# FoundationVision/OmniTokenizer

Measured on NVIDIA H100. Metric: video_frames_per_sec_encode_decode, higher is better.
Workload: dtype f32

## Files before the change

omnitokenizer_b200/_cabi.py:

```python
from __future__ import annotations

import ctypes
import os
from ctypes import c_char_p, c_float, c_int, c_int64, c_void_p, POINTER

import torch

_LIB_NAME = "libomnitok_b200.so"
_lib = None

EPI_NONE, EPI_GEGLU, EPI_QKV, EPI_QKV_PLANES = 0, 1, 2, 3
MATH_FP32, MATH_3XTF32, MATH_F16X1, MATH_F16X3 = 0, 1, 2, 3
ABI_VERSION = 2


class LinearHArgs(ctypes.Structure):
    _fields_ = [("a_hi", c_void_p), ("a_lo", c_void_p), ("a_rs", c_void_p), ("a2_rs", c_void_p), ("w_scale", c_float),
                ("a2_hi", c_void_p), ("a2_lo", c_void_p), ("n_split", c_int),
                ("lda", c_int), ("a_seg", c_int), ("a_seg_stride", c_int), ("a_seg_off", c_int),
                ("w_hi", c_void_p), ("w_lo", c_void_p),
                ("c", c_void_p), ("ldc", c_int), ("c_seg", c_int), ("c_seg_stride", c_int), ("c_seg_off", c_int),
                ("u_hi", c_void_p), ("u_lo", c_void_p), ("ldu", c_int),
                ("M", c_int), ("N", c_int), ("K", c_int),
                ("bias", c_void_p), ("residual", c_void_p), ("ldr", c_int),
                ("epilogue", c_int),
                ("q_scale", c_void_p), ("k_scale", c_void_p), ("rope_cos", c_void_p), ("rope_sin", c_void_p),
                ("qk_cols", c_int), ("tokens", c_int),
                ("q_plane_scale", c_float), ("k_plane_scale", c_float), ("vinv", c_void_p),
                ("a_rs_uniform", c_float), ("u_scale", c_float)]


SIGNATURES = {
    "omt_abi_version": (c_int, []),
    "omt_last_error": (c_char_p, []),
    "omt_device_info": (c_int, [POINTER(c_int)] * 3),
    "omt_set_option": (c_int, [c_char_p, c_int]),
    "omt_linear": (c_int, [c_void_p, c_int, c_int, c_int, c_int, c_void_p, c_void_p, c_void_p, c_int, c_int, c_int,
                           c_int, c_int, c_int, c_int, c_void_p, c_void_p, c_int, c_int, c_int, c_void_p]),
    "omt_linear2": (c_int, [c_void_p, c_void_p, c_int, c_int, c_void_p, c_void_p, c_void_p, c_int, c_int, c_int, c_int,
                            c_int, c_void_p, c_void_p, c_void_p, c_void_p, c_int, c_int, c_void_p]),
    "omt_linear_h": (c_int, [POINTER(LinearHArgs), c_void_p]),
    "omt_linear_h1": (c_int, [POINTER(LinearHArgs), c_void_p]),
    "omt_layernorm": (c_int, [c_void_p, c_int, c_void_p, c_int, c_void_p, c_void_p, c_int, c_int, c_float, c_int, c_int,
                              c_int, c_void_p]),
    "omt_layernorm_h": (c_int, [c_void_p, c_int, c_void_p, c_int, c_void_p, c_void_p, c_void_p, c_void_p, c_void_p, c_void_p,
                                c_int, c_void_p, c_void_p, c_int, c_int, c_float, c_int, c_int, c_int, c_void_p]),
    "omt_patchify_ln": (c_int, [c_void_p, c_void_p, c_void_p, c_void_p, c_void_p, c_void_p, c_void_p] + [c_int] * 8 + [c_float, c_void_p]),
    "omt_patchify_ln_u8": (c_int, [c_void_p] * 9 + [c_int] * 8 + [c_float, c_void_p]),
    "omt_u8_norm_select": (c_int, [c_void_p, c_int, c_int64, c_void_p, c_void_p]),
    "omt_resample_u8": (c_int, [c_void_p, c_int64, c_void_p, c_void_p, c_void_p, c_void_p, c_int64, c_int, c_int, c_int,
                                c_void_p, c_void_p]),
    "omt_resample_clips": (c_int, [c_void_p, c_int64, c_void_p, c_void_p, c_void_p, c_void_p, c_int64, c_void_p, c_int,
                                   c_int, c_int, c_int, c_void_p, c_void_p]),
    "omt_fvd_preprocess": (c_int, [c_void_p, c_int64, c_void_p, c_void_p, c_void_p, c_void_p, c_int64, c_void_p,
                                   c_void_p, c_int, c_int, c_int, c_int, c_void_p, c_void_p]),
    "omt_fvd_suite_preprocess": (c_int, [c_void_p, c_int64, c_int, c_int, c_void_p, c_void_p, c_void_p, c_void_p,
                                         c_int64, c_int, c_int, c_int, c_int, c_void_p, c_void_p]),
    "omt_conv3d": (c_int, [c_void_p, c_int, c_int, c_int, c_int, c_int, c_void_p, c_void_p, c_int, c_void_p]
                   + [c_int] * 13 + [c_void_p, c_int, c_int, c_void_p]),
    "omt_maxpool3d": (c_int, [c_void_p] + [c_int] * 17 + [c_void_p, c_void_p]),
    "omt_i3d_head": (c_int, [c_void_p, c_int, c_int, c_int, c_int, c_void_p, c_void_p, c_int, c_void_p, c_void_p]),
    "omt_fid_preprocess": (c_int, [c_void_p, c_int64, c_void_p, c_void_p, c_void_p, c_void_p, c_int64, c_void_p,
                                   c_void_p, c_int, c_int, c_int, c_void_p, c_void_p]),
    "omt_pool2d": (c_int, [c_void_p] + [c_int] * 13 + [c_void_p, c_int, c_int, c_void_p]),
    "omt_psnr_ssim": (c_int, [c_void_p] * 6 + [c_int] * 4 + [c_void_p] * 4),
    "omt_lpips_input": (c_int, [c_void_p] * 4 + [c_int] * 4 + [c_void_p, c_void_p]),
    "omt_lpips_head": (c_int, [c_void_p] + [c_int] * 5 + [c_void_p, c_int, c_void_p, c_void_p, c_void_p]),
    "omt_unpatchify": (c_int, [c_void_p, c_void_p] + [c_int] * 8 + [c_void_p]),
    "omt_unpatchify_u8": (c_int, [c_void_p, c_void_p] + [c_int] * 8 + [c_float] * 5 + [c_void_p]),
    "omt_peg": (c_int, [c_void_p, c_void_p, c_void_p, c_void_p, c_void_p, c_int, c_int, c_int, c_void_p]),
    "omt_peg_volume": (c_int, [c_void_p, c_void_p, c_void_p, c_void_p] + [c_int] * 7 + [c_void_p]),
    "omt_peg_volume_varlen": (c_int, [c_void_p] * 6 + [c_int] * 7 + [c_void_p]),
    "omt_qk_prep": (c_int, [c_void_p, c_int, c_void_p, c_int, c_void_p, c_void_p, c_void_p, c_void_p, c_int, c_int,
                            c_int, c_void_p]),
    "omt_attn_spatial": (c_int, [c_void_p, c_int, c_void_p, c_int, c_void_p, c_int, c_void_p, c_void_p, c_void_p, c_int,
                                 c_int, c_int, c_int, c_float, c_void_p]),
    "omt_attn_spatial_h": (c_int, [c_void_p, c_void_p, c_int, c_void_p, c_void_p, c_int, c_void_p, c_void_p, c_int, c_void_p,
                                   c_float, c_void_p, c_void_p, c_void_p, c_int, c_int, c_int, c_int, c_float, c_void_p]),
    "omt_attn_spatial_h1": (c_int, [c_void_p, c_int, c_void_p, c_int, c_void_p, c_int, c_void_p, c_float, c_void_p, c_void_p,
                                    c_int, c_int, c_int, c_int, c_float, c_void_p]),
    "omt_attn_window": (c_int, [c_void_p, c_int, c_void_p, c_int, c_void_p, c_int, c_void_p, c_void_p, c_void_p, c_int,
                                c_void_p, c_int, c_int, c_int, c_int, c_int, c_float, c_void_p]),
    "omt_attn_temporal": (c_int, [c_void_p, c_int, c_void_p, c_int, c_void_p, c_int, c_void_p, c_void_p, c_void_p, c_int,
                                  c_int, c_int, c_int, c_int, c_float, c_int, c_void_p]),
    "omt_attn_temporal_varlen": (c_int, [c_void_p, c_int, c_void_p, c_int, c_void_p, c_int, c_void_p, c_void_p, c_void_p,
                                         c_int, c_void_p, c_void_p, c_int, c_int, c_int, c_int, c_float, c_int, c_void_p]),
    "omt_pre_vq": (c_int, [c_void_p, c_int, c_void_p, c_void_p, c_void_p, c_int, c_int, c_int, c_int, c_void_p]),
    "omt_vq_search": (c_int, [c_void_p, c_void_p, c_void_p, c_int, c_int, c_void_p, c_void_p, c_void_p]),
    "omt_vq_fused": (c_int, [c_void_p, c_int, c_void_p, c_void_p, c_int, c_int, c_void_p, c_void_p, c_void_p, c_int, c_int,
                             c_void_p, c_void_p, c_void_p]),
    "omt_post_vq": (c_int, [c_void_p] * 8 + [c_int, c_int, c_int, c_void_p]),
}


def lib_path() -> str:
    return os.environ.get("OMT_LIB") or os.path.join(os.path.dirname(os.path.abspath(__file__)), _LIB_NAME)


def load():
    global _lib
    if _lib is not None:
        return _lib
    path = lib_path()
    if not os.path.exists(path):
        raise RuntimeError(
            f"{path} not found: the CUDA extension is not built. Run `python -c 'import __graft_entry__ as g; "
            f"g.build()'` (or `make -C omnitokenizer_b200/csrc`). There is no CPU fallback.")
    lib = ctypes.CDLL(path)
    for name, (res, args) in SIGNATURES.items():
        fn = getattr(lib, name)
        fn.restype = res
        fn.argtypes = args
    if lib.omt_abi_version() != ABI_VERSION:
        raise RuntimeError("libomnitok_b200.so ABI version mismatch")
    _lib = lib
    return lib


def _ptr(t):
    if t is None:
        return None
    if isinstance(t, int):
        return t
    return t.data_ptr()


def _stream():
    return torch.cuda.current_stream().cuda_stream


KERNELS_PER_CALL = {"omt_u8_norm_select": 2}
launch_count = 0


def call(name: str, *args):
    global launch_count
    lib = load()
    launch_count += KERNELS_PER_CALL.get(name, 1)
    conv = [_ptr(a) if (a is None or isinstance(a, torch.Tensor)) else a for a in args]
    rc = getattr(lib, name)(*conv, _stream())
    if rc != 0:
        raise RuntimeError(f"{name} failed ({rc}): {lib.omt_last_error().decode()}")


def linear_h(name="omt_linear_h", **kw):
    global launch_count
    lib = load()
    a = LinearHArgs()
    for k, v in kw.items():
        setattr(a, k, _ptr(v) if (v is None or isinstance(v, torch.Tensor)) else v)
    launch_count += 1
    rc = getattr(lib, name)(ctypes.byref(a), _stream())
    if rc != 0:
        raise RuntimeError(f"{name} failed ({rc}): {lib.omt_last_error().decode()}")


DEFAULT_OPTIONS = {"attn_kernel": 3, "peg_kernel": 4, "f16_bn": 0, "attn_f16_ctas": 2}


def set_option(name: str, value: int):
    lib = load()
    rc = lib.omt_set_option(name.encode(), int(value))
    if rc != 0:
        raise RuntimeError(f"omt_set_option({name}) failed: {lib.omt_last_error().decode()}")


def device_info():
    lib = load()
    a, b, c = c_int(), c_int(), c_int()
    rc = lib.omt_device_info(ctypes.byref(a), ctypes.byref(b), ctypes.byref(c))
    if rc != 0:
        raise RuntimeError(lib.omt_last_error().decode())
    return a.value, b.value, c.value
```

omnitokenizer_b200/csrc/rowwise.cu:

```cuda
#include "omt_common.cuh"
#include <string.h>

namespace omt {

static thread_local char g_err[512] = "";

void set_error(const char* fmt, ...) {
  va_list ap;
  va_start(ap, fmt);
  vsnprintf(g_err, sizeof(g_err), fmt, ap);
  va_end(ap);
}

int g_peg_kernel = 4;
int g_pdl = 0;
static int g_dev_ok[64];
static int g_sms[64];

int check_device() {
  int dev = 0;
  OMT_CUDA(cudaGetDevice(&dev));
  if (dev < 0 || dev >= 64) { set_error("device ordinal %d out of range", dev); return OMT_E_ARG; }
  if (g_dev_ok[dev] == 0) {
    cudaDeviceProp p;
    OMT_CUDA(cudaGetDeviceProperties(&p, dev));
    g_sms[dev] = p.multiProcessorCount;
    g_dev_ok[dev] = (p.major == 9 && p.minor == 0) ? 1 : -1;
  }
  if (g_dev_ok[dev] < 0) {
    set_error("omnitok_b200 kernels are built for sm_90a (H100) only (no fallback path)");
    return OMT_E_ARCH;
  }
  return OMT_OK;
}

int sm_count() {
  int dev = 0;
  cudaGetDevice(&dev);
  return (dev >= 0 && dev < 64 && g_sms[dev] > 0) ? g_sms[dev] : 148;
}

struct LnPlanes {
  uint16_t* y_hi; uint16_t* y_lo;
  uint16_t* x_hi; uint16_t* x_lo;
  int lds;
  float* y_rs; float* x_rs;
};

template <int NV, bool PAIR>
__global__ void __launch_bounds__(256) layernorm_kernel(const float* __restrict__ x, int ldx,
                                                        float* __restrict__ y, int ldy,
                                                        const float* __restrict__ w,
                                                        const float* __restrict__ b, int M, int C,
                                                        float eps, int seg, int seg_stride, int seg_off,
                                                        const LnPlanes pl) {
  pdl_sync();
  const int lane = threadIdx.x & 31;
  const int lrow = blockIdx.x * (blockDim.x >> 5) + (threadIdx.x >> 5);
  if (lrow >= M) return;
  const long long row = map_row(lrow, seg, seg_stride, seg_off);
  const float* xr = x + (size_t)row * ldx;
  float4 v[NV];
  float s = 0.f;
#pragma unroll
  for (int i = 0; i < NV; ++i) {
    const int c = PAIR ? ((i >> 1) * 32 + lane) * 8 + (i & 1) * 4 : (i * 32 + lane) * 4;
    if (c < C) {
      v[i] = *reinterpret_cast<const float4*>(xr + c);
      s += (v[i].x + v[i].y) + (v[i].z + v[i].w);
      if (pl.x_hi != nullptr && pl.x_rs == nullptr) store_split4(pl.x_hi, pl.x_lo, (size_t)lrow * pl.lds + c, v[i]);
    } else {
      v[i] = make_float4(0.f, 0.f, 0.f, 0.f);
    }
  }
  if (pl.x_hi != nullptr && pl.x_rs != nullptr) {
    float mx = 0.f;
#pragma unroll
    for (int i = 0; i < NV; ++i) mx = fmaxf(mx, max4abs(v[i]));
    float sc, inv;
    row_scale(warp_max(mx), sc, inv);
    if constexpr (PAIR) {
#pragma unroll
      for (int i = 0; i < NV; i += 2) {
        const int c = ((i >> 1) * 32 + lane) * 8;
        if (c < C) store_split8u(pl.x_hi, pl.x_lo, (size_t)lrow * pl.lds + c, v[i], v[i + 1], sc);
      }
    } else {
#pragma unroll
      for (int i = 0; i < NV; ++i) {
        const int c = (i * 32 + lane) * 4;
        if (c < C) store_split4u(pl.x_hi, pl.x_lo, (size_t)lrow * pl.lds + c, v[i], sc);
      }
    }
    if (lane == 0) pl.x_rs[lrow] = inv;
  }
  const float mean = warp_sum(s) / (float)C;
  float q = 0.f;
#pragma unroll
  for (int i = 0; i < NV; ++i) {
    const int c = PAIR ? ((i >> 1) * 32 + lane) * 8 + (i & 1) * 4 : (i * 32 + lane) * 4;
    if (c < C) {
      v[i].x -= mean; v[i].y -= mean; v[i].z -= mean; v[i].w -= mean;
      q += (v[i].x * v[i].x + v[i].y * v[i].y) + (v[i].z * v[i].z + v[i].w * v[i].w);
    }
  }
  const float rstd = 1.0f / sqrtf(warp_sum(q) / (float)C + eps);
  float* yr = y + (size_t)row * ldy;
  float omx = 0.f;
#pragma unroll
  for (int i = 0; i < NV; ++i) {
    const int c = PAIR ? ((i >> 1) * 32 + lane) * 8 + (i & 1) * 4 : (i * 32 + lane) * 4;
    if (c < C) {
      const float4 g = *reinterpret_cast<const float4*>(w + c);
      float4 o;
      o.x = v[i].x * rstd * g.x; o.y = v[i].y * rstd * g.y;
      o.z = v[i].z * rstd * g.z; o.w = v[i].w * rstd * g.w;
      if (b != nullptr) {
        const float4 bb = *reinterpret_cast<const float4*>(b + c);
        o.x += bb.x; o.y += bb.y; o.z += bb.z; o.w += bb.w;
      }
      if (y != nullptr) *reinterpret_cast<float4*>(yr + c) = o;
      if (pl.y_hi != nullptr && pl.y_rs == nullptr) store_split4(pl.y_hi, pl.y_lo, (size_t)lrow * pl.lds + c, o);
      v[i] = o;
      omx = fmaxf(omx, max4abs(o));
    }
  }
  if (pl.y_hi != nullptr && pl.y_rs != nullptr) {
    float sc, inv;
    row_scale(warp_max(omx), sc, inv);
    if constexpr (PAIR) {
#pragma unroll
      for (int i = 0; i < NV; i += 2) {
        const int c = ((i >> 1) * 32 + lane) * 8;
        if (c < C) store_split8u(pl.y_hi, pl.y_lo, (size_t)lrow * pl.lds + c, v[i], v[i + 1], sc);
      }
    } else {
#pragma unroll
      for (int i = 0; i < NV; ++i) {
        const int c = (i * 32 + lane) * 4;
        if (c < C) store_split4u(pl.y_hi, pl.y_lo, (size_t)lrow * pl.lds + c, v[i], sc);
      }
    }
    if (lane == 0) pl.y_rs[lrow] = inv;
  }
}

struct PatchRow {
  int bi, t0, hi, wi;
};

__device__ __forceinline__ PatchRow patch_row(int row, int T, int H, int W, int p, int pt, int first) {
  const int hh = H / p, ww = W / p;
  int r = row;
  PatchRow pr;
  pr.wi = r % ww; r /= ww;
  pr.hi = r % hh; r /= hh;
  int ti = 0;
  if (!first) { const int tn = (T - 1) / pt; ti = r % tn; r /= tn; }
  pr.bi = r;
  pr.t0 = first ? 0 : 1 + ti * pt;
  return pr;
}

template <int NV>
__device__ __forceinline__ void patch_ln_emit(float4 (&v)[NV], int row, int K, int lane, float* __restrict__ A,
                                              uint16_t* __restrict__ A_hi, uint16_t* __restrict__ A_lo,
                                              float* __restrict__ A_rs, const float* __restrict__ lw,
// ... 343 lines not shown
#pragma unroll
  for (int r9 = 0; r9 < 9; ++r9) {
    const float* rp = tp + ((st + r9 / 3) * (HB + 2) + sh + r9 % 3) * RS;
    win[r9][1] = *reinterpret_cast<const float2*>(rp);
    win[r9][2] = *reinterpret_cast<const float2*>(rp + PEG_CC);
  }
  const int fbase = ((t0 + st) * h + (h0 + sh)) * w;
  int tau = fbase % T, nn = fbase / T;
  for (int w2 = 0; w2 < w; ++w2) {
    float2 acc = bb;
#pragma unroll
    for (int r9 = 0; r9 < 9; ++r9) {
      const float* rp = tp + ((st + r9 / 3) * (HB + 2) + sh + r9 % 3) * RS + (w2 + 2) * PEG_CC;
      win[r9][0] = win[r9][1]; win[r9][1] = win[r9][2];
      win[r9][2] = *reinterpret_cast<const float2*>(rp);
#pragma unroll
      for (int kw = 0; kw < 3; ++kw) {
        acc.x = fmaf(win[r9][kw].x, wt[r9 * 3 + kw].x, acc.x);
        acc.y = fmaf(win[r9][kw].y, wt[r9 * 3 + kw].y, acc.y);
      }
    }
    const float2 ctr = causal ? win[7][1] : win[4][1];
    acc.x += ctr.x; acc.y += ctr.y;
    const int row = temporal ? tau * N + nn : fbase + w2;
    *reinterpret_cast<float2*>(y + (bbase + row) * C + c0 + 2 * cp) = acc;
    if (++tau == T) { tau = 0; ++nn; }
  }
}

__device__ __forceinline__ float2 lds_f2(uint32_t addr) {
  float2 v;
  asm volatile("ld.shared.v2.f32 {%0, %1}, [%2];" : "=f"(v.x), "=f"(v.y) : "r"(addr));
  return v;
}
template <int R>
__device__ __forceinline__ float2 peg_step(float2 (&win)[9][3], const float2 (&wt)[27], const float2 bb,
                                           const uint32_t (&a)[9], const bool causal) {
  float2 acc = bb;
#pragma unroll
  for (int r9 = 0; r9 < 9; ++r9) {
    win[r9][(2 + R) % 3] = lds_f2(a[r9] + R * (PEG_CC * 4));
#pragma unroll
    for (int kw = 0; kw < 3; ++kw) acc = ffma2(win[r9][(kw + R) % 3], wt[r9 * 3 + kw], acc);
  }
  const float2 ctr = causal ? win[7][(1 + R) % 3] : win[4][(1 + R) % 3];
  acc.x += ctr.x; acc.y += ctr.y;
  return acc;
}

__global__ void __launch_bounds__(160, 3) peg_tile4_kernel(const float* __restrict__ x, float* __restrict__ y,
                                                           const float* __restrict__ w27,
                                                           const float* __restrict__ bias, int T, int h, int w,
                                                           int C, int temporal, int causal, int TT, int HB, int RS, int zrow,
                                                           const int32_t* __restrict__ t_off) {
  pdl_sync();
  extern __shared__ __align__(16) float tile[];
  const int N = h * w;
  const int n_hblk = (h + HB - 1) / HB;
  const int t0 = (blockIdx.x / n_hblk) * TT, h0 = (blockIdx.x % n_hblk) * HB;
  const int c0 = blockIdx.y * PEG_CC;
  long long bbase = (long long)blockIdx.z * T * N;
  if (t_off != nullptr) {
    const int f0 = t_off[blockIdx.z];
    T = t_off[blockIdx.z + 1] - f0;
    bbase = (long long)f0 * N;
    if (t0 >= T) return;
  }
  const int pad_lo = causal ? 2 : 1;
  const int rows = (TT + 2) * (HB + 2);
  const int lane = threadIdx.x & 31, warp = threadIdx.x >> 5, nwarps = blockDim.x >> 5;
  const uint32_t inv_T = (65536u + (uint32_t)T - 1u) / (uint32_t)T;
  const uint32_t tile_s = static_cast<uint32_t>(__cvta_generic_to_shared(tile));
  const int chunks = (w + 2) * 4;
  const int pz_lo = t0 < pad_lo ? pad_lo - t0 : 0;
  for (int i = threadIdx.x; i < RS / 4; i += blockDim.x)
    asm volatile("st.shared.v4.f32 [%0], {%1, %1, %1, %1};" ::"r"(tile_s + (uint32_t)(zrow * RS + 4 * i) * 4u), "f"(0.f) : "memory");
  for (int pr = warp; pr < rows; pr += nwarps) {
    const int ph = pr % (HB + 2), pt = pr / (HB + 2);
    const int t2 = t0 - pad_lo + pt, h2 = h0 - 1 + ph;
    if (t2 < 0 || t2 >= T) continue;
    const bool row_ok = h2 >= 0 && h2 < h;
    const int fb = row_ok ? (t2 * h + h2) * w : 0;
    const int tau0 = fb % T, nn0 = fb / T;
    const uint32_t dst_row = tile_s + (uint32_t)(((pt - pz_lo) * (HB + 2) + ph) * RS) * 4u;
    for (int j = lane; j < chunks; j += 32) {
      const int w2 = (j >> 2) - 1;
      const bool ok = row_ok && w2 >= 0 && w2 < w;
      long long row = 0;
      if (ok) {
        if (temporal) {
          const uint32_t v = (uint32_t)(tau0 + w2);
          const uint32_t q = (v * inv_T) >> 16;
          row = (long long)(v - q * (uint32_t)T) * N + nn0 + (int)q;
        } else {
          row = fb + w2;
        }
      }
      const float* src = x + (bbase + row) * C + c0 + (j & 3) * 4;
      asm volatile("cp.async.cg.shared.global [%0], [%1], 16, %2;" ::"r"(dst_row + (uint32_t)j * 16u), "l"(src), "r"(ok ? 16 : 0) : "memory");
    }
  }
  asm volatile("cp.async.commit_group;" ::: "memory");
  const int cp = threadIdx.x & 7;
  const int strip = threadIdx.x >> 3;
  const int sh = strip % HB, st = strip / HB;
  const bool active = st < TT && t0 + st < T && h0 + sh < h;
  float2 wt[27];
  float2 bb = make_float2(0.f, 0.f);
  if (active) {
#pragma unroll
    for (int k = 0; k < 27; ++k) wt[k] = __ldg(reinterpret_cast<const float2*>(w27 + (size_t)k * C + c0 + 2 * cp));
    bb = __ldg(reinterpret_cast<const float2*>(bias + c0 + 2 * cp));
  }
  asm volatile("cp.async.wait_group 0;" ::: "memory");
  __syncthreads();
  if (!active) return;
  uint32_t a[9];
#pragma unroll
  for (int r9 = 0; r9 < 9; ++r9) {
    const int pt = st + r9 / 3;
    const int t2 = t0 - pad_lo + pt;
    const int prow = (t2 < 0 || t2 >= T) ? zrow : (pt - pz_lo) * (HB + 2) + sh + r9 % 3;
    a[r9] = tile_s + (uint32_t)((prow * RS + 2 * cp) * 4);
  }
  float2 win[9][3];
#pragma unroll
  for (int r9 = 0; r9 < 9; ++r9) {
    win[r9][0] = lds_f2(a[r9]);
    win[r9][1] = lds_f2(a[r9] + PEG_CC * 4);
    a[r9] += 2 * PEG_CC * 4;
  }
  const int fbase = ((t0 + st) * h + (h0 + sh)) * w;
  int tau = fbase % T;
  const long long row0 = temporal ? (long long)tau * N + fbase / T : (long long)fbase;
  float* yp = y + (bbase + row0) * C + c0 + 2 * cp;
  const long long inc = temporal ? (long long)N * C : (long long)C;
  const long long wrap = (long long)T * N * C - C;
  const bool cz = causal != 0;
#define OMT_PEG_STEP(R)                                                                             \
  {                                                                                                 \
    const float2 acc = peg_step<R>(win, wt, bb, a, cz);                                             \
    *reinterpret_cast<float2*>(yp) = acc;                                                           \
    yp += inc;                                                                                      \
    if (temporal && ++tau == T) { tau = 0; yp -= wrap; }                                            \
  }
  for (int wb = 0; wb < w; wb += 3) {
    OMT_PEG_STEP(0)
    if (wb + 1 < w) OMT_PEG_STEP(1)
    if (wb + 2 < w) OMT_PEG_STEP(2)
#pragma unroll
    for (int r9 = 0; r9 < 9; ++r9) a[r9] += 3 * PEG_CC * 4;
  }
#undef OMT_PEG_STEP
}

__device__ __forceinline__ void qk_prep_one(float* p, const float2 cs, bool rope, const float2 sc) {
  float2 v = *reinterpret_cast<float2*>(p);
  if (rope) {
    const float a = v.x * cs.x - v.y * cs.y;
    const float b = v.x * cs.y + v.y * cs.x;
    v.x = a; v.y = b;
  }
  const float ss = warp_sum(v.x * v.x + v.y * v.y);
  const float den = fmaxf(sqrtf(ss), 1e-12f);
  v.x = v.x / den * sc.x;
  v.y = v.y / den * sc.y;
  *reinterpret_cast<float2*>(p) = v;
}

__global__ void __launch_bounds__(256) qk_prep_kernel(float* __restrict__ q, int ldq,
                                                      float* __restrict__ k, int ldk,
                                                      const float* __restrict__ qs,
                                                      const float* __restrict__ ks,
                                                      const float* __restrict__ rc,
                                                      const float* __restrict__ rs, int M, int N,
                                                      int heads) {
  pdl_sync();
  const int lane = threadIdx.x & 31;
  const int row = blockIdx.x * (blockDim.x >> 5) + (threadIdx.x >> 5);
  if (row >= M) return;
  const bool rope = rc != nullptr;
  float2 cs = make_float2(1.f, 0.f);
  if (rope) {
    const int pos = row % N;
    cs.x = rc[pos * 32 + lane];
    cs.y = rs[pos * 32 + lane];
  }
  const float2 sq = *reinterpret_cast<const float2*>(qs + 2 * lane);
  const float2 sk = *reinterpret_cast<const float2*>(ks + 2 * lane);
  for (int h = 0; h < heads; ++h) {
    qk_prep_one(q + (size_t)row * ldq + h * 64 + 2 * lane, cs, rope, sq);
    qk_prep_one(k + (size_t)row * ldk + h * 64 + 2 * lane, cs, rope, sk);
  }
}

}

using namespace omt;

extern "C" int omt_abi_version(void) { return OMT_ABI_VERSION; }
extern "C" const char* omt_last_error(void) { return omt::g_err; }

extern "C" int omt_device_info(int* sms, int* major, int* minor) {
  int dev = 0;
  OMT_CUDA(cudaGetDevice(&dev));
  cudaDeviceProp p;
  OMT_CUDA(cudaGetDeviceProperties(&p, dev));
  if (sms) *sms = p.multiProcessorCount;
  if (major) *major = p.major;
  if (minor) *minor = p.minor;
  return OMT_OK;
}

static int layernorm_impl(const char* who, const float* x, int ldx, float* y, int ldy, const omt::LnPlanes& pl, const float* w,
                          const float* b, int M, int C, float eps, int seg, int seg_stride, int seg_off, omt_stream_t stream) {
  OMT_ENTER();
  OMT_REQUIRE(x && w && (y || pl.y_hi), "%s: null pointer", who);
  OMT_REQUIRE(M >= 0 && C > 0 && C % 4 == 0 && C <= 1024, "%s: C=%d must be a multiple of 4, <= 1024", who, C);
  OMT_REQUIRE(ldx % 4 == 0 && ldx >= C && (y == nullptr || (ldy % 4 == 0 && ldy >= C)), "%s: bad leading dims", who);
  OMT_REQUIRE(aligned_to(16, {x, y, w, b}), "%s: x, y, w and b must be 16-byte aligned", who);
  OMT_REQUIRE((pl.y_hi == nullptr) == (pl.y_lo == nullptr) && (pl.x_hi == nullptr) == (pl.x_lo == nullptr), "%s: planes come in hi / lo pairs", who);
  if (pl.y_hi != nullptr || pl.x_hi != nullptr) {
    OMT_REQUIRE(pl.lds % 4 == 0 && pl.lds >= C, "%s: plane leading dimension %d", who, pl.lds);
    OMT_REQUIRE(((uintptr_t)pl.y_hi | (uintptr_t)pl.y_lo | (uintptr_t)pl.x_hi | (uintptr_t)pl.x_lo) % 8 == 0, "%s: planes must be 8-byte aligned", who);
  }
  if (M == 0) return OMT_OK;
  cudaStream_t st = (cudaStream_t)stream;
  const int nv = (C / 4 + 31) / 32;
  const bool pair = C % 256 == 0 && pl.lds % 8 == 0 &&
                    ((uintptr_t)pl.y_hi | (uintptr_t)pl.y_lo | (uintptr_t)pl.x_hi | (uintptr_t)pl.x_lo) % 16 == 0;
  dim3 grid((M + 7) / 8), block(256);
  switch (nv) {
    case 1: OMT_CUDA(launch_k(layernorm_kernel<1, false>, grid, block, 0, st, x, ldx, y, ldy, w, b, M, C, eps, seg, seg_stride, seg_off, pl)); break;
    case 2:
      if (pair) OMT_CUDA(launch_k(layernorm_kernel<2, true>, grid, block, 0, st, x, ldx, y, ldy, w, b, M, C, eps, seg, seg_stride, seg_off, pl));
      else OMT_CUDA(launch_k(layernorm_kernel<2, false>, grid, block, 0, st, x, ldx, y, ldy, w, b, M, C, eps, seg, seg_stride, seg_off, pl));
      break;
    case 3: OMT_CUDA(launch_k(layernorm_kernel<3, false>, grid, block, 0, st, x, ldx, y, ldy, w, b, M, C, eps, seg, seg_stride, seg_off, pl)); break;
    case 4:
      if (pair) OMT_CUDA(launch_k(layernorm_kernel<4, true>, grid, block, 0, st, x, ldx, y, ldy, w, b, M, C, eps, seg, seg_stride, seg_off, pl));
      else OMT_CUDA(launch_k(layernorm_kernel<4, false>, grid, block, 0, st, x, ldx, y, ldy, w, b, M, C, eps, seg, seg_stride, seg_off, pl));
      break;
    case 6:
      if (pair) OMT_CUDA(launch_k(layernorm_kernel<6, true>, grid, block, 0, st, x, ldx, y, ldy, w, b, M, C, eps, seg, seg_stride, seg_off, pl));
      else OMT_CUDA(launch_k(layernorm_kernel<8, false>, grid, block, 0, st, x, ldx, y, ldy, w, b, M, C, eps, seg, seg_stride, seg_off, pl));
      break;
    case 8:
      if (pair) OMT_CUDA(launch_k(layernorm_kernel<8, true>, grid, block, 0, st, x, ldx, y, ldy, w, b, M, C, eps, seg, seg_stride, seg_off, pl));
      else OMT_CUDA(launch_k(layernorm_kernel<8, false>, grid, block, 0, st, x, ldx, y, ldy, w, b, M, C, eps, seg, seg_stride, seg_off, pl));
      break;
    default: OMT_CUDA(launch_k(layernorm_kernel<8, false>, grid, block, 0, st, x, ldx, y, ldy, w, b, M, C, eps, seg, seg_stride, seg_off, pl)); break;
  }
  OMT_LAUNCH_CHECK();
  return OMT_OK;
}

extern "C" int omt_layernorm(const float* x, int ldx, float* y, int ldy, const float* w, const float* b,
                             int M, int C, float eps, int seg, int seg_stride, int seg_off,
                             omt_stream_t stream) {
  OMT_REQUIRE(y != nullptr, "omt_layernorm: null pointer");
  omt::LnPlanes pl{nullptr, nullptr, nullptr, nullptr, 0, nullptr, nullptr};
  return layernorm_impl("omt_layernorm", x, ldx, y, ldy, pl, w, b, M, C, eps, seg, seg_stride, seg_off, stream);
}

extern "C" int omt_layernorm_h(const float* x, int ldx, float* y, int ldy, uint16_t* y_hi, uint16_t* y_lo, float* y_rs,
                               uint16_t* x_hi, uint16_t* x_lo, float* x_rs, int lds, const float* w, const float* b,
                               int M, int C, float eps, int seg, int seg_stride, int seg_off, omt_stream_t stream) {
  OMT_REQUIRE((y_rs == nullptr || y_hi != nullptr) && (x_rs == nullptr || x_hi != nullptr), "omt_layernorm_h: row scales without planes");
  omt::LnPlanes pl{y_hi, y_lo, x_hi, x_lo, lds, y_rs, x_rs};
  return layernorm_impl("omt_layernorm_h", x, ldx, y, ldy, pl, w, b, M, C, eps, seg, seg_stride, seg_off, stream);
}

extern "C" int omt_patchify_ln(const float* video, float* A, uint16_t* A_hi, uint16_t* A_lo, float* A_rs, const float* ln_w,
                               const float* ln_b, int B, int Cin, int T, int H, int W, int p, int pt, int first,
                               float eps, omt_stream_t stream) {
  OMT_ENTER();
  OMT_REQUIRE(video && (A || A_hi) && ((ln_w == nullptr) == (ln_b == nullptr)) && ((A_hi == nullptr) == (A_lo == nullptr)),
              "omt_patchify_ln: null pointer");
  OMT_REQUIRE(aligned_to(16, {video, A, ln_w, ln_b}), "omt_patchify_ln: video, A, ln_w and ln_b must be 16-byte aligned");
  OMT_REQUIRE(((uintptr_t)A_hi | (uintptr_t)A_lo) % 8 == 0, "omt_patchify_ln: planes must be 8-byte aligned");
  OMT_REQUIRE(A_rs == nullptr || A_hi != nullptr, "omt_patchify_ln: row scales without planes");
  OMT_REQUIRE(p % 4 == 0 && H % p == 0 && W % p == 0, "omt_patchify_ln: patch %d must be a multiple of 4 dividing %dx%d", p, H, W);
  OMT_REQUIRE(first || (T > 1 && (T - 1) % pt == 0), "omt_patchify_ln: (T-1) %% pt != 0");
  const int PT = first ? 1 : pt;
  const int K = Cin * PT * p * p;
  OMT_REQUIRE(K <= 1024, "omt_patchify_ln: patch vector %d > 1024", K);
  const long long rows = (long long)B * (first ? 1 : (T - 1) / pt) * (H / p) * (W / p);
  if (rows == 0) return OMT_OK;
  cudaStream_t st = (cudaStream_t)stream;
  dim3 grid((unsigned)((rows + 7) / 8)), block(256);
  const int nv = (K / 4 + 31) / 32;
  if (nv <= 2)
    OMT_CUDA(launch_k(patchify_ln_kernel<2>, grid, block, 0, st, video, A, A_hi, A_lo, A_rs, ln_w, ln_b, (int)rows, Cin, T, H, W, p, pt, first, eps));
  else if (nv <= 6)
    OMT_CUDA(launch_k(patchify_ln_kernel<6>, grid, block, 0, st, video, A, A_hi, A_lo, A_rs, ln_w, ln_b, (int)rows, Cin, T, H, W, p, pt, first, eps));
  else
    OMT_CUDA(launch_k(patchify_ln_kernel<8>, grid, block, 0, st, video, A, A_hi, A_lo, A_rs, ln_w, ln_b, (int)rows, Cin, T, H, W, p, pt, first, eps));
  OMT_LAUNCH_CHECK();
  return OMT_OK;
}

extern "C" int omt_patchify_ln_u8(const uint8_t* frames, const float* lut, const int32_t* sel, float* A, uint16_t* A_hi,
                                  uint16_t* A_lo, float* A_rs, const float* ln_w, const float* ln_b, int B, int Cin, int T,
                                  int H, int W, int p, int pt, int first, float eps, omt_stream_t stream) {
  OMT_ENTER();
  OMT_REQUIRE(frames && lut && (A || A_hi) && ((ln_w == nullptr) == (ln_b == nullptr)) && ((A_hi == nullptr) == (A_lo == nullptr)),
              "omt_patchify_ln_u8: null pointer");
  OMT_REQUIRE(aligned_to(16, {A, ln_w, ln_b}), "omt_patchify_ln_u8: A, ln_w and ln_b must be 16-byte aligned");
  OMT_REQUIRE(((uintptr_t)A_hi | (uintptr_t)A_lo) % 8 == 0, "omt_patchify_ln_u8: planes must be 8-byte aligned");
  OMT_REQUIRE((uintptr_t)frames % 4 == 0, "omt_patchify_ln_u8: frames must be 4-byte aligned");
  OMT_REQUIRE(A_rs == nullptr || A_hi != nullptr, "omt_patchify_ln_u8: row scales without planes");
  OMT_REQUIRE(Cin >= 1 && Cin <= 4, "omt_patchify_ln_u8: Cin=%d must be 1..4", Cin);
  OMT_REQUIRE(p % 4 == 0 && p > 0 && H % p == 0 && W % p == 0, "omt_patchify_ln_u8: patch %d must be a multiple of 4 dividing %dx%d", p, H, W);
  OMT_REQUIRE(first || (T > 1 && pt > 0 && (T - 1) % pt == 0), "omt_patchify_ln_u8: (T-1) %% pt != 0");
  const int PT = first ? 1 : pt;
  const int K = Cin * PT * p * p;
  OMT_REQUIRE(K <= PU8_MAX_K, "omt_patchify_ln_u8: patch vector %d > %d", K, PU8_MAX_K);
  const long long rows = (long long)B * (first ? 1 : (T - 1) / pt) * (H / p) * (W / p);
  if (rows == 0) return OMT_OK;
  cudaStream_t st = (cudaStream_t)stream;
  long long blocks = (rows + PU8_WARPS - 1) / PU8_WARPS;
  if (blocks > (long long)sm_count() * 8) blocks = (long long)sm_count() * 8;
  dim3 grid((unsigned)blocks), block(32 * PU8_WARPS);
  const int nv = (K / 4 + 31) / 32;
  if (nv <= 2)
    OMT_CUDA(launch_k(patchify_ln_u8_kernel<2>, grid, block, 0, st, frames, lut, sel, A, A_hi, A_lo, A_rs, ln_w, ln_b, (int)rows, Cin, T, H, W, p, pt, first, eps));
  else if (nv <= 6)
    OMT_CUDA(launch_k(patchify_ln_u8_kernel<6>, grid, block, 0, st, frames, lut, sel, A, A_hi, A_lo, A_rs, ln_w, ln_b, (int)rows, Cin, T, H, W, p, pt, first, eps));
  else
    OMT_CUDA(launch_k(patchify_ln_u8_kernel<8>, grid, block, 0, st, frames, lut, sel, A, A_hi, A_lo, A_rs, ln_w, ln_b, (int)rows, Cin, T, H, W, p, pt, first, eps));
  OMT_LAUNCH_CHECK();
  return OMT_OK;
}

extern "C" int omt_u8_norm_select(const uint8_t* frames, int B, long long per_sample, int32_t* sel, omt_stream_t stream) {
  OMT_ENTER();
  OMT_REQUIRE(frames && sel, "omt_u8_norm_select: null pointer");
  OMT_REQUIRE(B >= 0 && B <= 65535 && per_sample >= 0, "omt_u8_norm_select: B=%d, per_sample=%lld", B, per_sample);
  if (B == 0) return OMT_OK;
  cudaStream_t st = (cudaStream_t)stream;
  OMT_CUDA(launch_k(u8_sel_init_kernel, dim3((B + 255) / 256), dim3(256), 0, st, sel, B));
  OMT_LAUNCH_CHECK();
  if (per_sample == 0) return OMT_OK;
  long long bx = (per_sample / 16 + 255) / 256;
  const long long cap = ((long long)sm_count() * 8 + B - 1) / B;
  if (bx > cap) bx = cap;
  if (bx < 1) bx = 1;
  OMT_CUDA(launch_k(u8_sel_scan_kernel, dim3((unsigned)bx, (unsigned)B), dim3(256), 0, st, frames, per_sample, sel));
  OMT_LAUNCH_CHECK();
  return OMT_OK;
}

extern "C" int omt_unpatchify(const float* P, float* video, int B, int Cin, int T, int H, int W, int p,
                              int pt, int first, omt_stream_t stream) {
  OMT_ENTER();
  OMT_REQUIRE(P && video, "omt_unpatchify: null pointer");
  OMT_REQUIRE(aligned_to(16, {P, video}), "omt_unpatchify: P and video must be 16-byte aligned");
  OMT_REQUIRE(p % 4 == 0 && H % p == 0 && W % p == 0, "omt_unpatchify: bad patch size");
  OMT_REQUIRE(first || (T > 1 && (T - 1) % pt == 0), "omt_unpatchify: (T-1) %% pt != 0");
  const int PT = first ? 1 : pt;
  const long long rows = (long long)B * (first ? 1 : (T - 1) / pt) * (H / p) * (W / p);
  const long long total4 = rows * (Cin * PT * p * p / 4);
  if (total4 == 0) return OMT_OK;
  long long blocks = (total4 + 255) / 256;
  if (blocks > 148LL * 32) blocks = 148LL * 32;
  OMT_CUDA(launch_k(unpatchify_kernel, dim3((unsigned)blocks), dim3(256), 0, (cudaStream_t)stream, P, video, total4, Cin, T, H, W, p, pt, first));
  OMT_LAUNCH_CHECK();
  return OMT_OK;
}

extern "C" int omt_unpatchify_u8(const float* P, uint8_t* out, int B, int Cin, int T, int H, int W, int p, int pt,
                                 int first, float mul, float add, float lo, float hi, float post, omt_stream_t stream) {
  OMT_ENTER();
  OMT_REQUIRE(P && out, "omt_unpatchify_u8: null pointer");
  OMT_REQUIRE(aligned_to(16, {P}), "omt_unpatchify_u8: P must be 16-byte aligned");
  OMT_REQUIRE(p % 4 == 0 && H % p == 0 && W % p == 0, "omt_unpatchify_u8: bad patch size");
  OMT_REQUIRE(first || (T > 1 && (T - 1) % pt == 0), "omt_unpatchify_u8: (T-1) %% pt != 0");
  OMT_REQUIRE(lo >= 0.f && hi * post < 256.f, "omt_unpatchify_u8: clamp range [%g, %g] x %g does not fit a byte", lo, hi, post);
  const int PT = first ? 1 : pt;
  const long long rows = (long long)B * (first ? 1 : (T - 1) / pt) * (H / p) * (W / p);
  const long long total = rows * PT * p * (p / 4);
  if (total == 0) return OMT_OK;
  long long blocks = (total + 255) / 256;
  if (blocks > 148LL * 32) blocks = 148LL * 32;
  OMT_CUDA(launch_k(unpatchify_u8_kernel, dim3((unsigned)blocks), dim3(256), 0, (cudaStream_t)stream, P, out, total, Cin, T, H, W, p,
                    pt, first, mul, add, lo, hi, post));
  OMT_LAUNCH_CHECK();
  return OMT_OK;
}

extern "C" int omt_peg(const float* x, float* y, const float* w27, const float* bias, const int32_t* nbr,
                       int B, int rows_per_b, int C, omt_stream_t stream) {
  OMT_ENTER();
  OMT_REQUIRE(x && y && w27 && bias && nbr, "omt_peg: null pointer");
  OMT_REQUIRE(x != y, "omt_peg: in-place is not supported (stencil)");
  OMT_REQUIRE(aligned_to(16, {x, y, w27, bias}), "omt_peg: x, y, w27 and bias must be 16-byte aligned");
  OMT_REQUIRE(C % 4 == 0 && C / 4 <= 128, "omt_peg: C=%d unsupported (need C %% 4 == 0, C <= 512)", C);
  const long long M = (long long)B * rows_per_b;
  if (M == 0) return OMT_OK;
  static bool attr_set[64];
  const size_t smem = (size_t)27 * C * sizeof(float);
  int dev0 = 0;
  cudaGetDevice(&dev0);
  if (dev0 >= 0 && dev0 < 64 && !attr_set[dev0]) {
    OMT_CUDA(cudaFuncSetAttribute(peg_kernel, cudaFuncAttributeMaxDynamicSharedMemorySize, 27 * 512 * 4));
    attr_set[dev0] = true;
  }
  const unsigned blocks = (unsigned)((M + PEG_ROWS - 1) / PEG_ROWS);
  peg_kernel<<<blocks, 128, smem, (cudaStream_t)stream>>>(x, y, w27, bias, nbr, rows_per_b, C, M);
  OMT_LAUNCH_CHECK();
  return OMT_OK;
}

static int peg_volume_launch(const char* who, const float* x, float* y, const float* w27, const float* bias,
                             const int32_t* t_off, int B, int T, int h, int w, int C, int temporal, int causal,
                             omt_stream_t stream) {
  OMT_REQUIRE(x && y && w27 && bias, "%s: null pointer", who);
  OMT_REQUIRE(x != y, "%s: in-place is not supported (stencil)", who);
  OMT_REQUIRE(aligned_to(16, {x}), "%s: x must be 16-byte aligned", who);
  OMT_REQUIRE(aligned_to(8, {y, w27, bias}), "%s: y, w27 and bias must be 8-byte aligned", who);
  OMT_REQUIRE(C % PEG_CC == 0 && C / PEG_CC <= 65535 && B <= 65535, "%s: C=%d must be a multiple of 16", who, C);
  OMT_REQUIRE(T >= 1 && h >= 1 && w >= 1, "%s: bad volume", who);
  if (B == 0) return OMT_OK;
  int RS = (w + 2) * PEG_CC;
  RS += ((16 - RS % 32) + 32) % 32;
  int TT = T < 5 ? T : 5, HB = 4;
  auto smem_of = [&](int tt, int hb) { return (size_t)(tt + 2) * (hb + 2) * (RS * sizeof(float) + (size_t)(w + 2) * 8); };
  while (HB > 1 && (smem_of(TT, HB) > 112 * 1024 || TT * HB * 8 > 256)) --HB;
  while (TT > 1 && (smem_of(TT, HB) > 112 * 1024 || TT * HB * 8 > 256)) --TT;
  const size_t smem = smem_of(TT, HB);
  OMT_REQUIRE(smem <= 200 * 1024, "%s: row of %d tokens does not fit the shared-memory tile", who, w);
  static size_t smem_set[64];
  int dev = 0;
  cudaGetDevice(&dev);
  if (dev >= 0 && dev < 64 && smem > smem_set[dev]) {
    OMT_CUDA(cudaFuncSetAttribute(peg_tile_kernel, cudaFuncAttributeMaxDynamicSharedMemorySize, (int)smem));
    smem_set[dev] = smem;
  }
  const int threads = ((TT * HB * 8 + 31) / 32) * 32;
  dim3 grid(((T + TT - 1) / TT) * ((h + HB - 1) / HB), C / PEG_CC, B);
  const bool fast_ok = T <= 64 && w <= 254;
  const bool v4 = g_peg_kernel == 4 && fast_ok;
  if (v4) {
    const int pad_lo = causal ? 2 : 1;
    int vp = 1;
    for (int t0 = 0; t0 < T; t0 += TT) {
      const int lo = t0 - pad_lo < 0 ? 0 : t0 - pad_lo, hi = t0 - pad_lo + TT + 2 > T ? T : t0 - pad_lo + TT + 2;
      if (hi - lo > vp) vp = hi - lo;
    }
    const int zrow = vp * (HB + 2);
    const size_t smem4 = (size_t)(zrow + 1) * RS * sizeof(float);
    static size_t smem4_set[64];
    if (dev >= 0 && dev < 64 && smem4 > smem4_set[dev]) {
      OMT_CUDA(cudaFuncSetAttribute(peg_tile4_kernel, cudaFuncAttributeMaxDynamicSharedMemorySize, (int)smem4));
      smem4_set[dev] = smem4;
    }
    OMT_CUDA(launch_k(peg_tile4_kernel, grid, dim3(threads), smem4, (cudaStream_t)stream, x, y, w27, bias, T, h, w, C, temporal, causal, TT, HB, RS, zrow, t_off));
  } else {
    OMT_CUDA(launch_k(peg_tile_kernel, grid, dim3(threads), smem, (cudaStream_t)stream, x, y, w27, bias, T, h, w, C, temporal, causal, TT, HB, RS, t_off));
  }
  OMT_LAUNCH_CHECK();
  return OMT_OK;
}

extern "C" int omt_peg_volume(const float* x, float* y, const float* w27, const float* bias, int B, int T, int h,
                              int w, int C, int temporal, int causal, omt_stream_t stream) {
  OMT_ENTER();
  return peg_volume_launch("omt_peg_volume", x, y, w27, bias, nullptr, B, T, h, w, C, temporal, causal, stream);
}

extern "C" int omt_peg_volume_varlen(const float* x, float* y, const float* w27, const float* bias, const int32_t* t_off_host,
                                     const int32_t* t_off, int B, int M, int h, int w, int C, int temporal, int causal,
                                     omt_stream_t stream) {
  OMT_ENTER();
  int t_max = 0;
  const int rc = check_t_off("omt_peg_volume_varlen", t_off_host, t_off, B, M, (long long)h * w, &t_max);
  if (rc) return rc;
  return peg_volume_launch("omt_peg_volume_varlen", x, y, w27, bias, t_off, B, t_max < 1 ? 1 : t_max, h, w, C, temporal,
                           causal, stream);
}

extern "C" int omt_qk_prep(float* q, int ldq, float* k, int ldk, const float* q_scale, const float* k_scale,
                           const float* rope_cos, const float* rope_sin, int M, int N, int heads,
                           omt_stream_t stream) {
  OMT_ENTER();
  OMT_REQUIRE(q && k && q_scale && k_scale, "omt_qk_prep: null pointer");
  OMT_REQUIRE((rope_cos == nullptr) == (rope_sin == nullptr), "omt_qk_prep: cos/sin must both be given");
  OMT_REQUIRE(ldq % 2 == 0 && ldk % 2 == 0 && N > 0, "omt_qk_prep: bad leading dims");
  OMT_REQUIRE(aligned_to(8, {q, k, q_scale, k_scale}), "omt_qk_prep: q, k, q_scale and k_scale must be 8-byte aligned");
  if (M == 0) return OMT_OK;
  OMT_CUDA(launch_k(qk_prep_kernel, dim3((M + 7) / 8), dim3(256), 0, (cudaStream_t)stream, q, ldq, k, ldk, q_scale, k_scale,
                    rope_cos, rope_sin, M, N, heads));
  OMT_LAUNCH_CHECK();
  return OMT_OK;
}

namespace omt { extern int g_attn_kernel; extern int g_f16_bn; extern int g_attn_f16_ctas; }

extern "C" int omt_set_option(const char* name, int value) {
  if (name == nullptr) return OMT_E_ARG;
  if (strcmp(name, "pdl") == 0) { omt::g_pdl = value ? 1 : 0; return OMT_OK; }
  if (strcmp(name, "peg_kernel") == 0) {
    if (value != 3 && value != 4) { omt::set_error("peg_kernel must be 3 or 4"); return OMT_E_ARG; }
    omt::g_peg_kernel = value;
    return OMT_OK;
  }
  if (strcmp(name, "attn_kernel") == 0) {
    if (value != 1 && value != 3) { omt::set_error("attn_kernel must be 1 or 3"); return OMT_E_ARG; }
    omt::g_attn_kernel = value;
    return OMT_OK;
  }
  if (strcmp(name, "f16_bn") == 0) {
    if (value != 0 && value != 128 && value != 256) { omt::set_error("f16_bn must be 0, 128 or 256"); return OMT_E_ARG; }
    omt::g_f16_bn = value;
    return OMT_OK;
  }
  if (strcmp(name, "attn_f16_ctas") == 0) {
    if (value != 1 && value != 2) { omt::set_error("attn_f16_ctas must be 1 or 2"); return OMT_E_ARG; }
    omt::g_attn_f16_ctas = value;
    return OMT_OK;
  }
  omt::set_error("unknown option %s", name);
  return OMT_E_ARG;
}
```

Baseline: 4155.

## Add register-blocked PEG depthwise conv kernel with cp.async row pipeline

Adds a new 3x3x3 depthwise PEG conv kernel (version 5) and makes it the default. Each thread computes 8 consecutive width outputs, reusing a 10-wide register window of shared-memory loads. Input rows are streamed into a 5-slot ring buffer with cp.async so loads overlap compute while the block walks down the height dimension. It adds register pressure and more complex index math for the temporal layout, and changes tile shapes and occupancy.

New measurement: 4174, median of 6. About the same (+0.5%).

```diff
diff --git a/omnitokenizer_b200/_cabi.py b/omnitokenizer_b200/_cabi.py
--- a/omnitokenizer_b200/_cabi.py
+++ b/omnitokenizer_b200/_cabi.py
@@ -155,7 +155,7 @@
         raise RuntimeError(f"{name} failed ({rc}): {lib.omt_last_error().decode()}")
 
 
-DEFAULT_OPTIONS = {"attn_kernel": 3, "peg_kernel": 4, "f16_bn": 0, "attn_f16_ctas": 2}
+DEFAULT_OPTIONS = {"attn_kernel": 3, "peg_kernel": 5, "f16_bn": 0, "attn_f16_ctas": 2}
 
 
 def set_option(name: str, value: int):
diff --git a/omnitokenizer_b200/csrc/rowwise.cu b/omnitokenizer_b200/csrc/rowwise.cu
--- a/omnitokenizer_b200/csrc/rowwise.cu
+++ b/omnitokenizer_b200/csrc/rowwise.cu
@@ -12,7 +12,7 @@
   va_end(ap);
 }
 
-int g_peg_kernel = 4;
+int g_peg_kernel = 5;
 int g_pdl = 0;
 static int g_dev_ok[64];
 static int g_sms[64];
@@ -662,6 +662,146 @@
     for (int r9 = 0; r9 < 9; ++r9) a[r9] += 3 * PEG_CC * 4;
   }
 #undef OMT_PEG_STEP
+}
+
+constexpr int PEG5_WS = 8;
+constexpr int PEG5_NSEG = 4;
+constexpr int PEG5_WC = PEG5_WS * PEG5_NSEG;
+constexpr int PEG5_TT = 5;
+constexpr int PEG5_HB = 32;
+constexpr int PEG5_NR = 5;
+constexpr int PEG5_PS = 624;
+__host__ __device__ constexpr int peg5_col(int c) { return (c + (c >> 3)) * PEG_CC; }
+
+__global__ void __launch_bounds__(PEG5_TT * PEG5_NSEG * PEG_CC, 2)
+peg_tile5_kernel(const float* __restrict__ x, float* __restrict__ y, const float* __restrict__ w27,
+                 const float* __restrict__ bias, int T, int h, int w, int C, int temporal, int causal, int TT, int HB,
+                 int VP, const int32_t* __restrict__ t_off) {
+  pdl_sync();
+  extern __shared__ __align__(16) float tile[];
+  const int nslab = C / PEG_CC, nwc = (w + PEG5_WC - 1) / PEG5_WC, nhb = (h + HB - 1) / HB;
+  int bx = blockIdx.x;
+  const int c0 = (bx % nslab) * PEG_CC;
+  bx /= nslab;
+  const int w0 = (bx % nwc) * PEG5_WC;
+  bx /= nwc;
+  const int h0 = (bx % nhb) * HB, t0 = (bx / nhb) * TT;
+  const int N = h * w;
+  long long bbase = (long long)blockIdx.z * T * N;
+  if (t_off != nullptr) {
+    const int f0 = t_off[blockIdx.z];
+    T = t_off[blockIdx.z + 1] - f0;
+    bbase = (long long)f0 * N;
+    if (t0 >= T) return;
+  }
+  const int pad_lo = causal ? 2 : 1;
+  const int tlo = t0 - pad_lo < 0 ? 0 : t0 - pad_lo;
+  const int nvp = (t0 - pad_lo + TT + 2 < T ? t0 - pad_lo + TT + 2 : T) - tlo;
+  const int nr = h - h0 < HB ? h - h0 : HB;
+  const int lane = threadIdx.x & 31, warp = threadIdx.x >> 5, nwarps = blockDim.x >> 5;
+  const uint32_t inv_T = (65536u + (uint32_t)T - 1u) / (uint32_t)T;
+  const uint32_t tile_s = static_cast<uint32_t>(__cvta_generic_to_shared(tile));
+  const int zrow = PEG5_NR * VP * PEG5_PS;
+  for (int i = threadIdx.x; i < PEG5_PS / 4; i += blockDim.x)
+    asm volatile("st.shared.v4.f32 [%0], {%1, %1, %1, %1};" ::"r"(tile_s + (uint32_t)(zrow + 4 * i) * 4u), "f"(0.f) : "memory");
+  auto gather = [&](int r) {
+    const int h2 = h0 - 1 + r;
+    if (r < nr + 2 && h2 >= 0 && h2 < h) {
+      const uint32_t dst = tile_s + (uint32_t)((r % PEG5_NR) * VP * PEG5_PS) * 4u;
+      for (int p = warp; p < nvp; p += nwarps) {
+        const int fb = ((tlo + p) * h + h2) * w;
+        const int tau0 = fb % T, nn0 = fb / T;
+        for (int j = lane; j < (PEG5_WC + 2) * 4; j += 32) {
+          const int c = j >> 2, w2 = w0 - 1 + c;
+          const bool ok = w2 >= 0 && w2 < w;
+          long long row = 0;
+          if (ok) {
+            if (temporal) {
+              const uint32_t v = (uint32_t)(tau0 + w2);
+              const uint32_t q = (v * inv_T) >> 16;
+              row = (long long)(v - q * (uint32_t)T) * N + nn0 + (int)q;
+            } else {
+              row = fb + w2;
+            }
+          }
+          const float* src = x + (bbase + row) * C + c0 + (j & 3) * 4;
+          const uint32_t d = dst + (uint32_t)(p * PEG5_PS + peg5_col(c) + (j & 3) * 4) * 4u;
+          asm volatile("cp.async.cg.shared.global [%0], [%1], 16, %2;" ::"r"(d), "l"(src), "r"(ok ? 16 : 0) : "memory");
+        }
+      }
+    }
+    asm volatile("cp.async.commit_group;" ::: "memory");
+  };
+#pragma unroll 1
+  for (int r = 0; r < PEG5_NR - 1; ++r) gather(r);
+  const int cl = threadIdx.x & 15, pl = (threadIdx.x >> 4) % TT, seg = (threadIdx.x >> 4) / TT;
+  const int t = t0 + pl, wbase = w0 + seg * PEG5_WS;
+  const bool active = t < T && wbase < w;
+  float wt[27];
+  float bb = 0.f;
+  if (active) {
+#pragma unroll
+    for (int k = 0; k < 27; ++k) wt[k] = __ldg(w27 + (size_t)k * C + c0 + cl);
+    bb = __ldg(bias + c0 + cl);
+  }
+  int pv[3];
+#pragma unroll
+  for (int dt = 0; dt < 3; ++dt) {
+    const int t2 = t - pad_lo + dt;
+    pv[dt] = t2 >= 0 && t2 < T ? t2 - tlo : -1;
+  }
+  const int lofs = peg5_col(seg * PEG5_WS) + cl;
+  int fb = (t * h + h0) * w + wbase;
+  int tau = fb % T, nn = fb / T;
+  const int wq = w / T, wr = w % T;
+  const long long inc = temporal ? (long long)N * C : (long long)C;
+  const long long wrap = (long long)T * N * C - C;
+#pragma unroll 1
+  for (int i = 0; i < nr; ++i) {
+    asm volatile("cp.async.wait_group %0;" ::"n"(PEG5_NR - 4) : "memory");
+    __syncthreads();
+    gather(i + PEG5_NR - 1);
+    if (active) {
+      int ao[9];
+#pragma unroll
+      for (int dh = 0; dh < 3; ++dh) {
+        const int h2 = h0 - 1 + i + dh;
+        const int sb = ((i + dh) % PEG5_NR) * VP;
+#pragma unroll
+        for (int dt = 0; dt < 3; ++dt)
+          ao[dt * 3 + dh] = (h2 >= 0 && h2 < h && pv[dt] >= 0 ? (sb + pv[dt]) * PEG5_PS : zrow) + lofs;
+      }
+      float acc[PEG5_WS], ctr[PEG5_WS];
+#pragma unroll
+      for (int j = 0; j < PEG5_WS; ++j) acc[j] = bb;
+#pragma unroll
+      for (int r9 = 0; r9 < 9; ++r9) {
+        float v[PEG5_WS + 2];
+#pragma unroll
+        for (int c = 0; c < PEG5_WS + 2; ++c) v[c] = tile[ao[r9] + peg5_col(c)];
+#pragma unroll
+        for (int j = 0; j < PEG5_WS; ++j)
+#pragma unroll
+          for (int kw = 0; kw < 3; ++kw) acc[j] = fmaf(v[j + kw], wt[r9 * 3 + kw], acc[j]);
+        if (r9 == (causal ? 7 : 4)) {
+#pragma unroll
+          for (int j = 0; j < PEG5_WS; ++j) ctr[j] = v[j + 1];
+        }
+      }
+      float* yp = y + (bbase + (temporal ? (long long)tau * N + nn : (long long)fb)) * C + c0 + cl;
+      int tj = tau;
+#pragma unroll
+      for (int j = 0; j < PEG5_WS; ++j) {
+        if (wbase + j < w) *yp = acc[j] + ctr[j];
+        yp += inc;
+        if (temporal && ++tj == T) { tj = 0; yp -= wrap; }
+      }
+    }
+    fb += w;
+    tau += wr;
+    nn += wq;
+    if (tau >= T) { tau -= T; ++nn; }
+  }
 }
 
 __device__ __forceinline__ void qk_prep_one(float* p, const float2 cs, bool rope, const float2 sc) {
@@ -950,8 +1090,25 @@
   const int threads = ((TT * HB * 8 + 31) / 32) * 32;
   dim3 grid(((T + TT - 1) / TT) * ((h + HB - 1) / HB), C / PEG_CC, B);
   const bool fast_ok = T <= 64 && w <= 254;
-  const bool v4 = g_peg_kernel == 4 && fast_ok;
-  if (v4) {
+  if (g_peg_kernel == 5 && fast_ok) {
+    const int ntb = (T + PEG5_TT - 1) / PEG5_TT, TT5 = (T + ntb - 1) / ntb, HB5 = h < PEG5_HB ? h : PEG5_HB;
+    const int pad_lo = causal ? 2 : 1;
+    int vp = 1;
+    for (int t0 = 0; t0 < T; t0 += TT5) {
+      const int lo = t0 - pad_lo < 0 ? 0 : t0 - pad_lo, hi = t0 - pad_lo + TT5 + 2 > T ? T : t0 - pad_lo + TT5 + 2;
+      if (hi - lo > vp) vp = hi - lo;
+    }
+    const size_t smem5 = (size_t)(PEG5_NR * vp + 1) * PEG5_PS * sizeof(float);
+    const long long nblk = (long long)(C / PEG_CC) * ((w + PEG5_WC - 1) / PEG5_WC) * ((h + HB5 - 1) / HB5) * ((T + TT5 - 1) / TT5);
+    OMT_REQUIRE(nblk <= 0x7fffffffLL, "%s: volume too large for one launch", who);
+    static size_t smem5_set[64];
+    if (dev >= 0 && dev < 64 && smem5 > smem5_set[dev]) {
+      OMT_CUDA(cudaFuncSetAttribute(peg_tile5_kernel, cudaFuncAttributeMaxDynamicSharedMemorySize, (int)smem5));
+      smem5_set[dev] = smem5;
+    }
+    OMT_CUDA(launch_k(peg_tile5_kernel, dim3((unsigned)nblk, 1, B), dim3(TT5 * PEG5_NSEG * PEG_CC), smem5, (cudaStream_t)stream, x, y,
+                      w27, bias, T, h, w, C, temporal, causal, TT5, HB5, vp, t_off));
+  } else if (g_peg_kernel == 4 && fast_ok) {
     const int pad_lo = causal ? 2 : 1;
     int vp = 1;
     for (int t0 = 0; t0 < T; t0 += TT) {
@@ -1011,7 +1168,7 @@
   if (name == nullptr) return OMT_E_ARG;
   if (strcmp(name, "pdl") == 0) { omt::g_pdl = value ? 1 : 0; return OMT_OK; }
   if (strcmp(name, "peg_kernel") == 0) {
-    if (value != 3 && value != 4) { omt::set_error("peg_kernel must be 3 or 4"); return OMT_E_ARG; }
+    if (value < 3 || value > 5) { omt::set_error("peg_kernel must be 3, 4 or 5"); return OMT_E_ARG; }
     omt::g_peg_kernel = value;
     return OMT_OK;
   }
```
